# Slienteagle-wyb/tdmpc

Measured on AMD Instinct MI355X. Metric: plan-steps/sec (N=512, H=5, iters=6) at 1/2/4/8 MI355X vs CPU ref, higher is better.
Workload: dtype fp32

## Files before the change

### tdmpc_amd/csrc/tdmpc_kernels.hip

```cpp
#include <hip/hip_runtime.h>
#include <hiprand/hiprand_kernel.h>

#include <math.h>
#include <stdint.h>
#include <stdio.h>
#include <stdlib.h>
#include <string.h>
#include <unistd.h>

#include <algorithm>
#include <atomic>
#include <chrono>
#include <mutex>
#include <type_traits>
#include <vector>

#include "../../include/tdmpc_hip.h"

typedef float floatx16 __attribute__((ext_vector_type(16)));

#define DEVI __device__ __forceinline__

#ifdef TDMPC_STAMPS
__device__ unsigned long long* g_stamps;
// ... 180 lines not shown

constexpr int SPLIT_S = 4;
constexpr int SPLIT_MAX_ROWS = 4096;

struct Work {
    float* X;
    float* H1;
    float* H2;
    float2* st1;
    float2* st2;
    float* rpart;
    float* G;
    float* rlast;
    float* value;
    float* qv;
    float* z0c;
    float* pimu;
    float* zpart;
    float* rpart_s;
    int split_rows;
    float* z0;
    float* mean;
    float* stdv;
    float* enc_tmp;
    size_t x_stride;
    int xrows;
    char* p1;
    size_t p1_bytes;
    size_t total;
};

size_t pixel_act_floats(const Layout& w) {
    size_t m = 0;
    for (int i = 1; i <= 4; ++i) m = std::max(m, (size_t)w.nch * w.conv_hw[i] * w.conv_hw[i]);
    return m;
}

constexpr int P1_NG = 8;
constexpr int P1_WPG = 32;
constexpr int P1_RTM = 3;
constexpr int P1_ROWS = 32 * P1_RTM;
constexpr int P1_H1LD = 544;
constexpr unsigned P1_XCC_TAB = P1_NG * 256 + 256;
constexpr unsigned P1_SPIN_MAX = 400000;

struct P1Region {
// ... 51 lines not shown
    const size_t M = w.M;
    size_t o = 0;
    auto take = [&](size_t bytes) { size_t r = o; o += rup(bytes, 256); return base ? base + r : nullptr; };
    k->xrows = (int)rup(B * T, 32);
    k->x_stride = (size_t)k->xrows * w.Kx;
    k->X = (float*)take((H + 1) * k->x_stride * 4);
    k->H1 = (float*)take((size_t)k->xrows * 2 * M * 4);
    k->H2 = (float*)take((size_t)k->xrows * 2 * M * 4);
    k->st1 = (float2*)take(B * T * (2 * M / 64) * 8);
    k->st2 = (float2*)take(B * T * (2 * M / 64) * 8);
    k->rpart = (float*)take(B * T * (M / 32) * 4);
    k->G = (float*)take(B * T * 4);
    k->rlast = (float*)take(B * T * 4);
    k->value = (float*)take(B * T * 4);
    k->qv = (float*)take(2 * (size_t)k->xrows * 4);
    k->pimu = (float*)take((size_t)k->xrows * w.Ap * 4);
    k->z0c = (float*)take(B * 2 * M * 4);
    k->split_rows = std::min(k->xrows, SPLIT_MAX_ROWS);
    k->zpart = (float*)take((size_t)2 * SPLIT_S * k->split_rows * std::max(w.Lr, w.Ar) * 4);
    k->rpart_s = (float*)take((size_t)2 * SPLIT_S * k->split_rows * 4);
    k->z0 = (float*)take(B * w.Lp * 4);
    k->mean = (float*)take(B * H * w.A * 4);
    k->stdv = (float*)take(B * H * w.A * 4);
    k->enc_tmp = (float*)take(d->modality ? 2 * B * pixel_act_floats(w) * 4 : 256);
    k->p1_bytes = p1_dims_ok(d, w) && !extra ? p1_region(d, w).total : 0;
    k->p1 = k->p1_bytes ? (char*)take(k->p1_bytes) : nullptr;
    k->total = o;
}

size_t cem_lds_bytes(int T, int H, int K, int A) {
    const size_t nl = (T + 63) / 64;
    return nl * 64 * 8 + ((size_t)H * K * A + 64 + 4 * rup((size_t)H * A, 4) + 64 + 32) * 4;
}

bool check_dims(const tdmpc_dims* d) {
    if (!d) return false;
    if (d->num_samples <= 0 || d->num_pi < 0 || d->num_elites <= 0 || d->max_horizon <= 0 ||
        d->max_horizon > 16 || d->max_iterations <= 0 || d->max_batch <= 0) return false;
    const int T = d->num_samples + d->num_pi;
    if (d->num_elites > T || d->num_elites > 64 || T > 4096) return false;
    Layout w;
    if (!make_layout(d, &w)) return false;
    if (w.Kx > 1024 || w.M > 1024 || w.L > 1024 || w.A > 256 || w.E > 1024) return false;
    if (cem_lds_bytes(T, d->max_horizon, d->num_elites, w.A) > 160 * 1024) return false;
    return true;
}
// ... 1802 lines not shown
    const int e = row / a.eps_G, rr = row % a.eps_G;
    const float* ep = a.eps + (size_t)e * a.eps_env + a.eps_off + (size_t)rr * a.A;
    float o[4];
#pragma unroll
    for (int cc = 0; cc < 4; ++cc) {
        const int col = 4 * q + cc;
        float x = 0.f;
        if (col < a.A) {
            float sv = a.part[(size_t)row * a.n3 + col];
#pragma unroll
            for (int sl = 1; sl < SPLIT_S; ++sl) sv += a.part[((size_t)sl * a.prow + row) * a.n3 + col];
            const float muv = tanhf(sv + a.b3[col]);
            x = muv;
            if (a.min_std > 0.f) {
                const float ee = tclamp(fmul(ep[col], a.min_std), -0.3f, 0.3f);
                x = tclamp(fadd(muv, ee), a.lo, a.hi);
            }
        }
        o[cc] = x;
    }
    *(float4*)(a.Xo + (size_t)(xr >> 5) * a.x_ts + (size_t)q * 128 + (xr & 31) * 4) = make_float4(o[0], o[1], o[2], o[3]);
}

__global__ void __launch_bounds__(256) z0c_kernel(const float* W1, const float* b1, const float* z0, int Kx, int Ap,
                                                   int Lp, int k1c, int M, float* out) {
    const int e = blockIdx.x, p = blockIdx.y, n = blockIdx.z * 256 + threadIdx.x;
    if (n >= M) return;
    const int nn = p * M + n;
    const float* wrow = W1 + (size_t)(nn >> 5) * Kx * 32 + (nn & 31) * 4;
    float acc = 0.f;
#pragma unroll 8
    for (int kq = k1c >> 2; kq < Kx >> 2; ++kq) {
        const float4 w = *(const float4*)(wrow + kq * 128);
        const int zi = 4 * kq - Ap;
        const float* zr = z0 + (size_t)e * Lp;
        acc = fmaf(w.x, zi + 0 < Lp ? zr[zi + 0] : 0.f, acc);
        acc = fmaf(w.y, zi + 1 < Lp ? zr[zi + 1] : 0.f, acc);
        acc = fmaf(w.z, zi + 2 < Lp ? zr[zi + 2] : 0.f, acc);
        acc = fmaf(w.w, zi + 3 < Lp ? zr[zi + 3] : 0.f, acc);
    }
    out[((size_t)e * 2 + p) * M + n] = acc + b1[nn];
}

struct PiMuArgs {
    int rows; RowMap amap; RowMap mmap; const float* mu; int Ap, A; float* Xo; long x_ts;
    const float* eps; int eps_G; long eps_env; long eps_off; float min_std, lo, hi;
};

DEVI void pi_from_mu_item(const PiMuArgs& a, long i) {
    const int nq = a.Ap / 4;
    const int row = (int)(i / nq), q = (int)(i % nq);
    if (row >= a.rows) return;
    const int xr = map_row(a.amap, row);
    const int e = row / a.eps_G, rr = row % a.eps_G;
    const float* ep = a.eps + (size_t)e * a.eps_env + a.eps_off + (size_t)rr * a.A;
    const float4 m = *(const float4*)(a.mu + (size_t)map_row(a.mmap, row) * a.Ap + 4 * q);
    const float mv[4] = {m.x, m.y, m.z, m.w};
    float o[4];
#pragma unroll
    for (int cc = 0; cc < 4; ++cc) {
        const int col = 4 * q + cc;
        float x = 0.f;
        if (col < a.A) {
            x = mv[cc];
// ... 104 lines not shown
    __syncthreads();
    if (tid < 32 && row < a.rows) {
        float q[2];
        for (int p = 0; p < 2; ++p) {
            float s = 0.f;
            for (int i = 0; i < 16; ++i) s += red[p][i][r];
            q[p] = s + a.b3[p];
        }
        const float qm = (q[0] != q[0] || q[1] != q[1]) ? NAN : fminf(q[0], q[1]);
        const int x = map_row(a.map, row);
        a.value[x] = nan_to_num(fadd(a.G[x], fmul(a.disc, qm)));
    }
}


struct PrepArgs {
    float* X; size_t x_stride; int Kx, apq, lpq;
    int B, N, T, H, A;
    const float* mean; const float* stdv; int mstride;
    const float* eps; long eps_env; long eps_off;
    const float* z0;
    long n_zq, n_sq;
    PiMuArgs pm; long n_pm;
};

__global__ void __launch_bounds__(256) prep_kernel(const PrepArgs a) {
    const long total = a.n_zq + a.n_sq + a.n_pm;
    for (long it = (long)blockIdx.x * blockDim.x + threadIdx.x; it < total; it += (long)gridDim.x * blockDim.x) {
        if (it >= a.n_zq + a.n_sq) {
            pi_from_mu_item(a.pm, it - a.n_zq - a.n_sq);
        } else if (it < a.n_zq) {
            const int row = (int)(it % a.T);
            const long r2 = it / a.T;
            const int q = (int)(r2 % a.lpq), e = (int)(r2 / a.lpq);
            const int gr = e * a.T + row;
            *(float4*)(a.X + (size_t)(gr >> 5) * a.Kx * 32 + (size_t)(a.apq + q) * 128 + (gr & 31) * 4) =
                *(const float4*)(a.z0 + (size_t)e * a.lpq * 4 + q * 4);
        } else {
            long r2 = it - a.n_zq;
            const int n = (int)(r2 % a.N); r2 /= a.N;
            const int q = (int)(r2 % a.apq); r2 /= a.apq;
            const int t = (int)(r2 % a.H);
            const int e = (int)(r2 / a.H);
            const float* mt = a.mean + (size_t)e * a.mstride + (size_t)t * a.A;
            const float* sd = a.stdv + (size_t)e * a.mstride + (size_t)t * a.A;
            const float* ep = a.eps + (size_t)e * a.eps_env + a.eps_off + ((size_t)t * a.N + n) * a.A;
            float v[4];
#pragma unroll
            for (int k = 0; k < 4; ++k) {
                const int cc = q * 4 + k;
                v[k] = cc < a.A ? tclamp(fadd(mt[cc], fmul(sd[cc], ep[cc])), -1.f, 1.f) : 0.f;
            }
// ... 46 lines not shown
                        const float ep = a.eps[(size_t)e * a.eps_env + a.reuse_off + ((size_t)t * a.E + j) * a.A + cc];
                        x = tclamp(fadd(mt[cc], fmul(sd[cc], ep)), -1.f, 1.f);
                    }
                }
                v[k] = x;
            }
        }
        const int gr = e * a.Tw + row;
        *(float4*)(a.X + (size_t)t * a.x_stride + (size_t)(gr >> 5) * a.Kx * 32 + (size_t)q * 128 + (gr & 31) * 4) =
            make_float4(v[0], v[1], v[2], v[3]);
    }
}

struct CemArgs {
    int final_iter, iter, H, N, P, T, A, K, Kx, Hmax, I;
    int Tw, NE, pi_base;
    float* elite_store;
    const float* X; size_t x_stride;
    const float* value;
    const float* G; const float* qv; int q_ld; float discH;
    float* value_out;
    const float* rlast;
    float* mean; float* stdv;
    const float* eps; long eps_env; long eps_cem_off; long eps_iter; long eps_act_off;
    const double* u;
    float* prev_mean; int eval_mode;
    float temperature, momentum, omm, std_floor;
    const float* std_floor_p;
    float* action; float* metrics;
    float* elite_out; float* score_out; float* mean_out; float* std_out;
    int no_pick; float* reward_out;
    const int* pstatus; int* status;
};

DEVI uint32_t f2ord(float v) {
    const uint32_t u = __float_as_uint(v);
    return (u & 0x80000000u) ? ~u : (u | 0x80000000u);
}
DEVI float ord2f(uint32_t o) { return __uint_as_float((o & 0x80000000u) ? (o & 0x7fffffffu) : ~o); }
DEVI unsigned long long topk_key(float v, int i) {
    return ((unsigned long long)(~f2ord(v)) << 32) | (unsigned)i;
}
DEVI float key_value(unsigned long long k) { return ord2f(~(uint32_t)(k >> 32)); }

DEVI unsigned long long shfl_xor_u64(unsigned long long v, int m) {
    const unsigned lo = __shfl_xor((unsigned)v, m, 64), hi = __shfl_xor((unsigned)(v >> 32), m, 64);
// ... 2 lines not shown
DEVI unsigned long long wave_sort64(unsigned long long key, int lane) {
    for (int k = 2; k <= 64; k <<= 1)
        for (int j = k >> 1; j > 0; j >>= 1) {
            const unsigned long long o = shfl_xor_u64(key, j);
            const bool up = (lane & k) == 0, lower = (lane & j) == 0;
            key = (lower == up) ? (key < o ? key : o) : (key > o ? key : o);
        }
    return key;
}
DEVI unsigned long long wave_clean64(unsigned long long key, int lane) {
    for (int j = 32; j > 0; j >>= 1) {
        const unsigned long long o = shfl_xor_u64(key, j);
        key = ((lane & j) == 0) ? (key < o ? key : o) : (key > o ? key : o);
    }
    return key;
}
DEVI float wave_sum(float v) {
    for (int off = 32; off > 0; off >>= 1) v += __shfl_xor(v, off, 64);
    return v;
}

DEVI int cem_row(const CemArgs& a, int c) { return c < a.NE ? c : a.pi_base + (c - a.NE); }

__global__ void __launch_bounds__(1024) cem_kernel(const CemArgs a) {
    extern __shared__ __attribute__((aligned(16))) float sm[];
    const int e = blockIdx.x, tid = threadIdx.x, nt = blockDim.x, lane = tid & 63, wave = tid >> 6;
    const int nwv = nt >> 6;
    const int H = a.H, A = a.A, K = a.K, T = a.T, N = a.N;
    const int HA = H * A, HKA = H * K * A;
    const int NL = (T + 63) / 64;
    unsigned long long* key = (unsigned long long*)sm;
    float* EA = (float*)(key + (size_t)NL * 64);
    float* sc = EA + HKA;
    float* omean = sc + 64;
    float* smean = omean + 2 * rup(HA, 4);
    float* sstd = smean + rup(HA, 4);
    int* eidx = (int*)(sstd + rup(HA, 4));
    float* red = (float*)(eidx + 64);
    float* gmean = a.mean + (size_t)e * a.Hmax * A;
    float* gstd = a.stdv + (size_t)e * a.Hmax * A;
    const float* val = a.value + (size_t)e * a.Tw;

    for (int i = tid; i < HA; i += nt) omean[i] = gmean[i];
    for (int l = wave; l < NL; l += nwv) {
        const int i = l * 64 + lane;
        float v = 0.f;
        if (i < T) {
            const int row = cem_row(a, i);
            if (a.qv) {
                const size_t x = (size_t)e * a.Tw + row;
                v = qvalue(a.G[x], a.qv[x], a.qv[a.q_ld + x], a.discH);
                if (a.value_out) a.value_out[((size_t)e * a.I + a.iter) * a.Tw + i] = v;
            } else {
                v = val[row];
                if (a.value_out) a.value_out[((size_t)e * a.I + a.iter) * a.Tw + i] = v;
            }
        }
        const unsigned long long k = i < T ? topk_key(v, i) : ~0ull;
        key[(size_t)l * 64 + lane] = wave_sort64(k, lane);
    }
    __syncthreads();
    for (int stride = 1; stride < NL; stride <<= 1) {
        for (int l = wave * 2 * stride; l < NL; l += nwv * 2 * stride) {
            if (l + stride < NL) {
                const unsigned long long x = key[(size_t)l * 64 + lane];
                const unsigned long long y = key[(size_t)(l + stride) * 64 + 63 - lane];
                key[(size_t)l * 64 + lane] = wave_clean64(x < y ? x : y, lane);
            }
        }
        __syncthreads();
    }
    if (tid < K) eidx[tid] = (int)(key[tid] & 0xffffffffu);
    __syncthreads();
    for (int base = 0; base < HKA; base += 8 * nt) {
        float v[8];
#pragma unroll
        for (int u = 0; u < 8; ++u) {
            const int idx = base + tid + u * nt;
            if (idx < HKA) {
                const int t = idx / (K * A), k = (idx / A) % K, c = idx % A;
                v[u] = a.X[(size_t)t * a.x_stride + pidx((size_t)e * a.Tw + cem_row(a, eidx[k]), c, a.Kx)];
            }
        }
#pragma unroll
        for (int u = 0; u < 8; ++u) {
            const int idx = base + tid + u * nt;
            if (idx < HKA) EA[idx] = v[u];
        }
    }
    if (wave == 0) {
        const float v0 = key_value(key[0]);
        float s = 0.f;
        if (lane < K) s = expf(fmul(a.temperature, key_value(key[lane]) - v0));
        const float tot = wave_sum(s);
        s = lane < K ? __fdiv_rn(s, tot) : 0.f;
        if (lane < 64) sc[lane] = s;
        const float tot2 = wave_sum(s);
        if (lane == 0) red[0] = fadd(tot2, 1e-9f);
    }
    __syncthreads();
    const float den = red[0];
    const float std_floor = a.std_floor_p ? *a.std_floor_p : a.std_floor;
    for (int i = tid; i < HA; i += nt) {
        const int t = i / A, c = i % A;
        const float* ea = EA + (size_t)t * K * A + c;
        float s = 0.f;
        for (int k = 0; k < K; ++k) s = fadd(s, fmul(sc[k], ea[(size_t)k * A]));
        const float mu = __fdiv_rn(s, den);
        float v = 0.f;
        for (int k = 0; k < K; ++k) {
            const float dd = ea[(size_t)k * A] - mu;
            v = fadd(v, fmul(sc[k], fmul(dd, dd)));
        }
        const float sd = tclamp(sqrtf(__fdiv_rn(v, den)), std_floor, 2.f);
        const float nm = fadd(fmul(a.momentum, omean[i]), fmul(a.omm, mu));
        smean[i] = nm; sstd[i] = sd;
        gmean[i] = nm; gstd[i] = sd;
        if (a.mean_out) a.mean_out[((size_t)e * a.I + a.iter) * HA + i] = nm;
        if (a.std_out) a.std_out[((size_t)e * a.I + a.iter) * HA + i] = sd;
    }
    if (a.elite_store)
        for (int i = tid; i < HKA; i += nt) a.elite_store[(size_t)e * a.Hmax * a.K * A + i] = EA[i];
    if (!a.final_iter) return;
    const int pst = a.pstatus ? *a.pstatus : 0;
    if (pst && tid == 0 && a.status)
        __hip_atomic_fetch_or(a.status, pst, __ATOMIC_RELAXED, __HIP_MEMORY_SCOPE_AGENT);
    if (a.elite_out)
        for (int i = tid; i < HKA; i += nt) a.elite_out[(size_t)e * HKA + i] = EA[i];
    if (a.score_out && tid < K) a.score_out[(size_t)e * K + tid] = sc[tid];
    {
        float s = 0.f;
        for (int i = tid; i < T; i += nt) s += a.rlast[(size_t)e * a.Tw + cem_row(a, i)];
        s = wave_sum(s);
        if (lane == 0) red[1 + wave] = s;
    }
    __syncthreads();
    if (a.no_pick) {
        if (tid == 0) {
            float rs = 0.f;
            for (int w = 0; w < nwv; ++w) rs += red[1 + w];
            a.reward_out[e] = rs / (float)T;
        }
        return;
    }
    int* jsel = (int*)(red + 20);
    if (tid == 0) {
        double last = 0.0;
        for (int k = 0; k < K; ++k) last += (double)sc[k];
        const double u = a.u[e];
        double acc = 0.0;
        int j = K - 1;
        for (int k = 0; k < K; ++k) {
            acc += (double)sc[k];
            if (acc / last > u) { j = k; break; }
        }
        *jsel = j;
        float rs = 0.f;
        for (int w = 0; w < nwv; ++w) rs += red[1 + w];
        float cs = 0.f;
        for (int c = 0; c < A; ++c) cs += sstd[c];
        a.metrics[(size_t)e * 2 + 0] = pst ? __builtin_nanf("") : rs / (float)T;
        a.metrics[(size_t)e * 2 + 1] = pst ? __builtin_nanf("") : cs / (float)A;
    }
    __syncthreads();
    const int j = *jsel;
    for (int c = tid; c < A; c += nt) {
        float v = EA[(size_t)j * A + c];
        if (!a.eval_mode) v = fadd(v, fmul(sstd[c], a.eps[(size_t)e * a.eps_env + a.eps_act_off + c]));
        if (pst) v = __builtin_nanf("");
        a.action[(size_t)e * A + c] = v;
        if (a.elite_store) a.elite_store[(size_t)e * a.Hmax * a.K * A + (size_t)j * A + c] = v;
    }
    for (int i = tid; i < HA; i += nt) a.prev_mean[(size_t)e * H * A + i] = smean[i];
}

struct EncArgs {
    const float* x; long x_stride; int xdim;
    int E, L, Lp;
    const float* w1t; const float* b1;
    const float* w2t; const float* b2;
    float* z0;
    float* mean; float* stdv; const float* prev_mean; int warm, H, A, Hmax;
    const int* warm_flags;
    const float* ln_g; const float* ln_b;
    int warm_keep_last;
    float init_std;
};

DEVI void enc_matvec(const float* wt, const float* in, int nin, int nout, float* part, int tid, int nt) {
    const int np = nt / nout > 0 ? nt / nout : 1;
    const int j = tid % nout, p = tid / nout;
    float s = 0.f;
    if (p < np && j < nout) {
#pragma unroll 8
        for (int k = p; k < nin; k += np) s += wt[(size_t)k * nout + j] * in[k];
    }
// ... 211 lines not shown
#define LDS_FOR_EACH(X) X(2, 1, 2, 4, 32) X(3, 1, 2, 4, 32) X(1, 1, 2, 2, 32)
#define CHAIN_FOR_EACH(X)                                                                            \
    X(CH_STEP, 1, 8, 4, 8, 0) X(CH_STEP, 2, 8, 4, 8, 0) X(CH_STEP, 4, 8, 4, 8, 0)                     \
    X(CH_PI, 1, 8, 4, 8, 0) X(CH_PI, 2, 8, 4, 8, 0) X(CH_PI, 4, 8, 4, 8, 0)                           \
    X(CH_Q, 1, 8, 4, 8, 0) X(CH_Q, 2, 8, 4, 8, 0) X(CH_Q, 4, 8, 4, 8, 0)                              \
    X(CH_STEP, 2, 8, 2, X6_D3, 1) X(CH_STEP, 4, 4, 2, 2, 1) X(CH_PI, 2, 8, 2, X6_D3, 1)               \
    X(CH_PI, 4, 4, 2, 2, 1) X(CH_Q, 2, 8, 2, X6_D3, 1) X(CH_Q, 4, 4, 2, 2, 1)
#define CHAIN16_FOR_EACH(X)                                                                          \
    X(CH_STEP, 2, 4, 4, 0) X(CH_STEP, 4, 4, 4, 0) X(CH_PI, 2, 4, 4, 0) X(CH_PI, 4, 4, 4, 0)           \
    X(CH_Q, 2, 4, 4, 0) X(CH_Q, 4, 4, 4, 0)                                                           \
    X(CH_STEP, 4, 4, 4, 1) X(CH_PI, 4, 4, 4, 1) X(CH_Q, 4, 4, 4, 1)
#define SPLIT_FOR_EACH(X) X(4, 4, 1) X(4, 4, 0)
#define CONV_TILE_FOR_EACH(X) X(1) X(2) X(4)
#define PLAN1_FOR_EACH(X) X(4) X(6)

int init_attrs() {
    static int done = 0;
    if (done) return 0;
    int rc = 0;
#define LINEAR_ATTR(...) rc |= set_max_lds<linear_kernel<__VA_ARGS__>>();
    FOR_EACH_LINEAR(LINEAR_ATTR)
#undef LINEAR_ATTR
    rc |= set_max_lds<cem_kernel>();
#define PLAN1_ATTR(KS) rc |= set_max_lds<plan1_kernel<KS>>();
    PLAN1_FOR_EACH(PLAN1_ATTR)
#undef PLAN1_ATTR
#define WIDE_ATTR(...) rc |= set_max_lds<wide_step_kernel<__VA_ARGS__>>();
    WIDE_FOR_EACH(WIDE_ATTR)
#undef WIDE_ATTR
#define WIDE_HEADS_ATTR(...) rc |= set_max_lds<wide_heads_kernel<__VA_ARGS__>>();
    WIDE_HEADS_FOR_EACH(WIDE_HEADS_ATTR)
#undef WIDE_HEADS_ATTR
    rc |= set_max_lds<qstat_chol_kernel>();
#define CONV_ATTR(PX) rc |= set_max_lds<conv_tile_kernel<PX>>();
    CONV_TILE_FOR_EACH(CONV_ATTR)
#undef CONV_ATTR
#define LDS_ATTR(...) rc |= set_max_lds<linear_lds_kernel<__VA_ARGS__, true>>() | set_max_lds<linear_lds_kernel<__VA_ARGS__, false>>();
    LDS_FOR_EACH(LDS_ATTR)
#undef LDS_ATTR
#define CHAIN_ATTR(...) rc |= set_max_lds<chain_kernel<__VA_ARGS__>>();
    CHAIN_FOR_EACH(CHAIN_ATTR)
#undef CHAIN_ATTR
#define CHAIN16_ATTR(...) rc |= set_max_lds<chain16_kernel<__VA_ARGS__>>();
    CHAIN16_FOR_EACH(CHAIN16_ATTR)
#undef CHAIN16_ATTR
    if (rc) return TDMPC_E_HIP;
// ... 327 lines not shown
    f.n3 = w.Lr; f.L = w.L; f.Lp = w.Lp; f.b3d = c.pw + w.b3d; f.b3r = c.pw + w.b3r;
    f.Xo = Xt(c, t + 1); f.x_ts = (long)c.Kx * 32; f.out_q0 = w.Ap / 4;
    f.G = c.k.G; f.rlast = c.k.rlast; f.disc = disc; f.first = first; f.last = last;
    const long nth = (long)rows * (w.Lp / 4 + 1);
    hipLaunchKernelGGL(split_finish_kernel, dim3((unsigned)((nth + 255) / 256)), dim3(256), 0, c.s, f);
    HIPCHK(hipGetLastError());
    return 0;
}

int flush_split(const Ctx& c) {
    if (!c.split_pend) return 0;
    c.split_pend = 0;
    const int par = 1 - c.split_par;
    const size_t zs = (size_t)SPLIT_S * c.k.split_rows * std::max(c.w.Lr, c.w.Ar), rs = (size_t)SPLIT_S * c.k.split_rows;
    return split_finish(c, c.split_t, c.split_rows, c.split_map, c.k.zpart + par * zs, c.k.rpart_s + par * rs,
                        c.split_disc, c.split_first, 0);
}

int z0c_k1c(const Ctx& c) { return (int)rup(c.w.Ap, 16); }
bool z0c_eligible(const Ctx& c) {
    static const int v = [] { const char* e = getenv("TDMPC_Z0C"); return e ? atoi(e) : 1; }();
    return v && z0c_k1c(c) < (int)rup(c.Kx, 16);
}
int z0c_launch(const Ctx& c) {
    hipLaunchKernelGGL(z0c_kernel, dim3(c.B, 2, (c.M + 255) / 256), dim3(256), 0, c.s, c.pw + c.w.w1x, c.pw + c.w.b1x,
                       c.k.z0, c.Kx, c.w.Ap, c.w.Lp, z0c_k1c(c), c.M, c.k.z0c);
    HIPCHK(hipGetLastError());
    return 0;
}

unsigned long long* g_p1_stamps = nullptr;

int wide_g1(const Ctx& c, bool z0c) {
    return (int)rup(z0c ? z0c_k1c(c) : c.Kx, 32) / 32;
}
bool wide_instance(int g1, int nb3, int mode) {
#define WIDE_HAS(G1, NB3, MODE) if (g1 == G1 && nb3 == NB3 && mode == (MODE)) return true;
    WIDE_FOR_EACH(WIDE_HAS)
#undef WIDE_HAS
    return false;
}
bool use_wide(const Ctx& c, int rows, const RowMap& map, bool z0c) {
    static const int en = [] { const char* e = getenv("TDMPC_WIDE"); return e ? atoi(e) : 1; }();
    if (c.w.M != 512 || !use_x6(c) || !num_cus()) return false;
    if (c.path != TDMPC_PATH_AUTO && c.path != TDMPC_PATH_CHAIN && c.path != TDMPC_PATH_WIDE) return false;
    if (c.path != TDMPC_PATH_WIDE && !en) return false;
    if (rows % 16 || map.G % 16 || map.S % 16 || map.O % 16) return false;
    if (z0c && map.G % 128) return false;
    const int g1 = wide_g1(c, z0c), nb3 = (int)rup(c.w.L, 16) / 16, mode = g1 > 5 ? WS_XS : 0;
    if (!wide_instance(g1, nb3, mode) || (c.w.fold && !wide_instance(g1, nb3, mode | WS_OUTH))) return false;
    return c.path == TDMPC_PATH_WIDE || (rows + 127) / 128 * 2 >= num_cus();
// ... 274 lines not shown

PiMuArgs pimu_args(const Ctx& c, int rows, RowMap map, const float* eps, long eps_env, int eps_G, long eps_off,
                   float min_std, float* Xo = nullptr, const RowMap* mmap = nullptr) {
    PiMuArgs f;
    memset(&f, 0, sizeof f);
    f.rows = rows; f.amap = map; f.mmap = mmap ? *mmap : map; f.mu = c.k.pimu; f.Ap = c.w.Ap; f.A = c.w.A;
    f.Xo = Xo ? Xo : Xt(c, c.H); f.x_ts = (long)c.Kx * 32;
    f.eps = eps; f.eps_G = eps_G; f.eps_env = eps_env; f.eps_off = eps_off; f.min_std = min_std;
    f.lo = (float)(-1.0 + 1e-6); f.hi = (float)(1.0 - 1e-6);
    return f;
}

int policy_from_mu(const Ctx& c, int rows, RowMap map, const float* eps, long eps_env, int eps_G, long eps_off,
                   float min_std, float* Xo = nullptr, const RowMap* mmap = nullptr) {
    const PiMuArgs f = pimu_args(c, rows, map, eps, eps_env, eps_G, eps_off, min_std, Xo, mmap);
    const long nth = (long)rows * (c.w.Ap / 4);
    if (!nth) return 0;
    hipLaunchKernelGGL(pi_from_mu_kernel, dim3((unsigned)((nth + 255) / 256)), dim3(256), 0, c.s, f);
    HIPCHK(hipGetLastError());
    return 0;
}

int prep_launch(const Ctx& c, const float* noise, int sample_rows, long eps_env, long eps_off, const float* z0,
                const PiMuArgs* pm) {
    PrepArgs a;
    memset(&a, 0, sizeof a);
    a.X = c.k.X; a.x_stride = c.k.x_stride; a.Kx = c.Kx; a.apq = c.w.Ap / 4; a.lpq = c.w.Lp / 4;
    a.B = c.B; a.N = sample_rows; a.T = c.T; a.H = c.H; a.A = c.A;
    a.mean = c.k.mean; a.stdv = c.k.stdv; a.mstride = c.d->max_horizon * c.A;
    a.eps = noise; a.eps_env = eps_env; a.eps_off = eps_off;
    a.z0 = z0;
    a.n_zq = z0 ? (long)c.B * a.lpq * c.T : 0;
    a.n_sq = noise ? (long)c.B * c.H * a.apq * sample_rows : 0;
    if (pm) {
        a.pm = *pm;
        a.n_pm = (long)pm->rows * (pm->Ap / 4);
    }
    const long total = a.n_zq + a.n_sq + a.n_pm;
    if (!total) return 0;
    const int blocks = (int)std::min<long>((total + 255) / 256, 2048);
    hipLaunchKernelGGL(prep_kernel, dim3(blocks), dim3(256), 0, c.s, a);
    HIPCHK(hipGetLastError());
    return 0;
}
int prep(const Ctx& c, const float* noise, int iter, const float* z0, const PiMuArgs* pm = nullptr) {
    return prep_launch(c, noise, c.N, c.eps_env, c.eps_cem_off + (long)iter * c.eps_iter, z0, pm);
}

int q_chain(const Ctx& c, int rows, RowMap map, const float* X = nullptr, float* qo = nullptr, int q_ld = 0,
            bool fold = false) {
    const Layout& w = c.w;
    const int M = c.M;
    ChainArgs a = chain0(c, rows, map, c.H, c.Kx, 0, 2);
    if (X) a.X = X;
    if (fold && !a.x6) {
        snprintf(g_err, sizeof g_err, "folded Q: chain x6 kernels only");
        return TDMPC_E_DIMS;
    }
    for (int q = 0; q < 2; ++q) {
        ChainProb& p = a.p[q];
        p.W1 = c.pw + w.wq1x + (size_t)q * M * c.Kx; p.b1 = c.pw + w.bq1x + q * M;
        p.g1 = c.pw + w.g1 + q * M; p.be1 = c.pw + w.be1 + q * M;
        p.W2 = c.pw + w.wq2 + (size_t)q * M * M; p.b2 = c.pw + w.bq2 + q * M;
        p.g2 = c.pw + w.g2 + q * M; p.be2 = c.pw + w.be2 + q * M;
        p.w3v = c.pw + w.wq3 + q * M; p.b3v = c.pw + w.bq3 + q;
        if (a.x6) {
            p.X1 = x6p(c, X6_WQ1X) + q * x6_w1_rows_stride(c);
            p.X2 = x6p(c, X6_WQ2) + (size_t)q * (M / 32) * (M / 16) * 1536;
        }
// ... 333 lines not shown
    return init_attrs();
}

int resolve_path(int path, bool whole_plan) {
    if (path < 0 || path > TDMPC_PATH_WIDE) { snprintf(g_err, sizeof g_err, "bad path"); return -1; }
    if (path == TDMPC_PATH_CHAIN64) return TDMPC_PATH_CHAIN_X6;
    return path == TDMPC_PATH_PERSIST && !whole_plan ? TDMPC_PATH_AUTO : path;
}

int load_z0(const Ctx& c, const float* z0) {
    const int L = c.w.L;
    hipLaunchKernelGGL(zero_words_kernel, dim3(1), dim3(256), 0, c.s, (unsigned*)c.k.z0, (int)((size_t)c.B * c.w.Lp));
    HIPCHK(hipGetLastError());
    HIPCHK(hipMemcpy2DAsync(c.k.z0, c.w.Lp * 4, z0, L * 4, L * 4, c.B, hipMemcpyDeviceToDevice, c.s));
    return prep(c, nullptr, 0, c.k.z0);
}

template <class Prm>
CemArgs cem_args(const Ctx& c, const Prm* prm, const float* eps, const double* u, float* prev_mean, float* action,
                 float* metrics, float* value_out, float* mean_out, float* std_out) {
    CemArgs ca;
    memset(&ca, 0, sizeof ca);
    ca.H = c.H; ca.N = c.N; ca.P = c.P; ca.T = ca.Tw = ca.NE = c.T; ca.A = c.A; ca.K = c.d->num_elites; ca.Kx = c.Kx;
    ca.Hmax = c.d->max_horizon; ca.mean = c.k.mean; ca.stdv = c.k.stdv; ca.pstatus = pack_status(c);
    ca.X = c.k.X; ca.x_stride = c.k.x_stride; ca.value = c.k.value; ca.rlast = c.k.rlast;
    ca.eps = eps; ca.u = u; ca.prev_mean = prev_mean;
    ca.eval_mode = prm->eval_mode; ca.temperature = prm->temperature; ca.momentum = prm->momentum;
    ca.omm = prm->one_minus_momentum; ca.std_floor = prm->std_floor; ca.action = action; ca.metrics = metrics;
    ca.value_out = value_out; ca.mean_out = mean_out; ca.std_out = std_out; ca.status = prm->status;
    return ca;
}
void cem_args_qv(CemArgs& ca, const Ctx& c, float discH) {
    ca.G = c.k.G; ca.qv = c.k.qv; ca.q_ld = c.k.xrows; ca.discH = discH;
}

struct ToldStep {
    const Ctx& c;
    int operator()(int t, int rows, RowMap map, float disc, int first, int last, int defer) const {
        return step_next(c, t, rows, map, disc, first, last, defer);
    }
};

struct PlanFast {
    bool z0c;
    bool fold;
    bool wide_heads;
    bool pi_cache;
};

template <class Step>
int cem_run(Ctx& c, const Step& step, const PlanFast& f, const tdmpc_plan_params* prm, const float* noise,
            const double* u, float* prev_mean, float* action, float* metrics, float* elite_out, float* score_out,
            float* value_out, float* mean_out, float* std_out) {
    int rc;
    const int H = c.H, I = prm->iterations, B = c.B, N = c.N, P = c.P, T = c.T;
    if ((rc = prep(c, noise, 0, c.k.z0))) return rc;
    if (f.z0c) {
        if ((rc = z0c_launch(c))) return rc;
        c.z0c_ready = 1;
    }
    if (f.fold) {
        const RowMap rm0 = {N, T, 0};
        c.fold_ok = c.w.fold && H > 1 && use_wide(c, B * N, rm0, c.z0c_ready != 0) && use_wide(c, B * N, rm0, false);
        c.fold_heads = c.fold_ok && !f.wide_heads && use_x6(c) && use_chain(c, B * N, 1, CK_PI) &&
                       use_chain(c, B * N, 2, CK_Q) && (P == 0 || use_chain(c, B * P, 2, CK_Q));
        if (c.fold_heads && P > 0 && use_chain(c, B * P, 2, CK_STEP) && use_chain(c, B * P, 1, CK_PI)) {
            const ChainArgs probe = chain0(c, B * P, RowMap{P, T, N}, 0, c.Kx, 0, 2);
            c.fold_policy = probe.rb == 32 && probe.x6;
        }
    }

    const RowMap all = {T, T, 0}, pm = {P, T, N}, rm = {N, T, 0};
    if (P > 0) {
        for (int t = 0; t < H; ++t) {
            if ((rc = policy(c, t, B * P, pm, noise, c.eps_env, P, (long)t * P * c.A, prm->min_std, nullptr,
                             c.fold_policy && t >= 1)))
                return rc;
            if ((rc = step(t, B * T, all, prm->discount_pow[t], t == 0, t == H - 1, 0))) return rc;
        }
    }
    CemArgs ca = cem_args(c, prm, noise, u, prev_mean, action, metrics, value_out, mean_out, std_out);
    ca.I = I; ca.std_floor_p = prm->std_floor_dev; ca.elite_out = elite_out; ca.score_out = score_out;
    ca.eps_env = c.eps_env; ca.eps_cem_off = c.eps_cem_off; ca.eps_iter = c.eps_iter; ca.eps_act_off = c.eps_act_off;
    if (f.wide_heads || c.fold_heads || use_chain(c, B * T, 2, CK_Q)) cem_args_qv(ca, c, prm->discount_pow[H]);
    const size_t cem_lds = cem_lds_bytes(T, H, ca.K, c.A);

    const bool pi_cache = f.pi_cache && P > 0 && use_chain(c, B * T, 1, CK_PI);
    for (int i = 0; i < I; ++i) {
        const long toff = c.eps_cem_off + (long)i * c.eps_iter + c.eps_term_off;
        if (i > 0) {
            const PiMuArgs pmu = pimu_args(c, B * P, pm, noise, c.eps_env, P, toff + (long)N * c.A, prm->min_std);
            if ((rc = prep(c, noise, i, nullptr, f.wide_heads && P > 0 ? &pmu : nullptr))) return rc;
        }
        if (i > 0 || P == 0)
            for (int t = 0; t < H; ++t)
                if ((rc = step(t, B * N, rm, prm->discount_pow[t], t == 0, t == H - 1, 1))) return rc;
        if (f.wide_heads) {
            if (P > 0) {
                if (i == 0) rc = policy(c, H, B * P, pm, noise, c.eps_env, P, toff + (long)N * c.A, prm->min_std, c.k.pimu);
                if (rc || (rc = flush_split(c))) return rc;
            }
            if ((rc = terminal_wide(c, noise, toff, prm->min_std))) return rc;
        } else if (c.fold_heads) {
            if ((rc = policy(c, H, B * N, rm, noise, c.eps_env, N, toff, prm->min_std, nullptr, true))) return rc;
            if (P > 0) {
                if (i == 0 || !pi_cache)
                    rc = policy(c, H, B * P, pm, noise, c.eps_env, P, toff + (long)N * c.A, prm->min_std,
                                pi_cache ? c.k.pimu : nullptr, c.fold_policy != 0);
                else
                    rc = policy_from_mu(c, B * P, pm, noise, c.eps_env, P, toff + (long)N * c.A, prm->min_std);
                if (rc) return rc;
            }
            if ((rc = q_chain(c, B * N, rm, nullptr, nullptr, 0, true))) return rc;
            if (P > 0 && (rc = q_chain(c, B * P, pm, nullptr, nullptr, 0, c.fold_policy != 0))) return rc;
        } else if (pi_cache && i > 0) {
            if ((rc = policy(c, H, B * N, rm, noise, c.eps_env, N, toff, prm->min_std))) return rc;
            if ((rc = flush_split(c))) return rc;
            if ((rc = policy_from_mu(c, B * P, pm, noise, c.eps_env, P, toff + (long)N * c.A, prm->min_std)))
                return rc;
        } else if ((rc = policy(c, H, B * T, all, noise, c.eps_env, T, toff, prm->min_std,
                                pi_cache ? c.k.pimu : nullptr))) {
            return rc;
        }
        if (!f.wide_heads && !c.fold_heads && (rc = terminal_q(c, prm->discount_pow[H]))) return rc;
        ca.final_iter = i == I - 1;
        ca.iter = i;
        hipLaunchKernelGGL(cem_kernel, dim3(B), dim3(1024), cem_lds, c.s, ca);
        HIPCHK(hipGetLastError());
    }
    return 0;
}

bool icem_counts_ok(const tdmpc_icem_params* prm, const tdmpc_dims* d, const char* who) {
    const int H = prm->horizon, I = prm->iterations, N = d->num_samples, K = d->num_elites, P0 = prm->n_pi0;
    if (I <= 0 || I > 16) { snprintf(g_err, sizeof g_err, "%s: 1..16 iterations", who); return false; }
    if (P0 <= 0 || P0 > d->num_pi || prm->n_samples[0] != N) {
        snprintf(g_err, sizeof g_err, "%s: bad counts", who);
        return false;
    }
    for (int i = 0; i < I; ++i) {
        const int Ni = prm->n_samples[i], Pi = prm->n_pi[i], Ei = prm->n_elite[i];
        if (Ni <= 0 || Ni > N || Pi <= 0 || Pi > P0 || Ei < 0 || Ei > K || Ni + Ei + Pi < K ||
            (Ei > 0 && i == 0 && !prm->has_elites) ||
            (i == 0 && Ei > 0 && prm->elite_horizon != H && prm->elite_horizon != H - 1)) {
            snprintf(g_err, sizeof g_err, "%s: bad counts at iteration %d", who, i);
            return false;
        }
    }
    return true;
}
// ... 478 lines not shown
```

Measured before the change: 6184.

## Fuse CEM refit with next-iteration sample prep and fold z0c into prep kernel

Adds a cem_prep_kernel that runs the CEM refit redundantly across several blocks per environment and then writes the next iteration's sampled actions (and policy-from-mu rows) into X. This removes the separate prep launch between iterations. The mean/std buffers are double-buffered so the old stats can be reread, and elite actions are recomputed from the old mean/std and eps instead of read from X. The z0c kernel becomes an item range inside prep_kernel, and the top-k merge goes from a 2-way to a 4-way tree. The cost is duplicated refit work per slice and extra LDS for the old std.

```diff
diff --git a/tdmpc_amd/csrc/tdmpc_kernels.hip b/tdmpc_amd/csrc/tdmpc_kernels.hip
--- a/tdmpc_amd/csrc/tdmpc_kernels.hip
+++ b/tdmpc_amd/csrc/tdmpc_kernels.hip
@@ -226,6 +226,8 @@
     float* z0;
     float* mean;
     float* stdv;
+    float* mean2;
+    float* stdv2;
     float* enc_tmp;
     size_t x_stride;
     int xrows;
@@ -323,6 +325,8 @@
     k->z0 = (float*)take(B * w.Lp * 4);
     k->mean = (float*)take(B * H * w.A * 4);
     k->stdv = (float*)take(B * H * w.A * 4);
+    k->mean2 = (float*)take(B * H * w.A * 4);
+    k->stdv2 = (float*)take(B * H * w.A * 4);
     k->enc_tmp = (float*)take(d->modality ? 2 * B * pixel_act_floats(w) * 4 : 256);
     k->p1_bytes = p1_dims_ok(d, w) && !extra ? p1_region(d, w).total : 0;
     k->p1 = k->p1_bytes ? (char*)take(k->p1_bytes) : nullptr;
@@ -2171,24 +2175,24 @@
     *(float4*)(a.Xo + (size_t)(xr >> 5) * a.x_ts + (size_t)q * 128 + (xr & 31) * 4) = make_float4(o[0], o[1], o[2], o[3]);
 }
 
-__global__ void __launch_bounds__(256) z0c_kernel(const float* W1, const float* b1, const float* z0, int Kx, int Ap,
-                                                   int Lp, int k1c, int M, float* out) {
-    const int e = blockIdx.x, p = blockIdx.y, n = blockIdx.z * 256 + threadIdx.x;
-    if (n >= M) return;
-    const int nn = p * M + n;
-    const float* wrow = W1 + (size_t)(nn >> 5) * Kx * 32 + (nn & 31) * 4;
+struct Z0cArgs { const float* W1; const float* b1; const float* z0; int Kx, Ap, Lp, k1c, M; float* out; };
+
+DEVI void z0c_item(const Z0cArgs& a, long i) {
+    const int n = (int)(i % a.M), p = (int)(i / a.M % 2), e = (int)(i / (2 * a.M));
+    const int nn = p * a.M + n;
+    const float* wrow = a.W1 + (size_t)(nn >> 5) * a.Kx * 32 + (nn & 31) * 4;
+    const float* zr = a.z0 + (size_t)e * a.Lp;
     float acc = 0.f;
 #pragma unroll 8
-    for (int kq = k1c >> 2; kq < Kx >> 2; ++kq) {
+    for (int kq = a.k1c >> 2; kq < a.Kx >> 2; ++kq) {
         const float4 w = *(const float4*)(wrow + kq * 128);
-        const int zi = 4 * kq - Ap;
-        const float* zr = z0 + (size_t)e * Lp;
-        acc = fmaf(w.x, zi + 0 < Lp ? zr[zi + 0] : 0.f, acc);
-        acc = fmaf(w.y, zi + 1 < Lp ? zr[zi + 1] : 0.f, acc);
-        acc = fmaf(w.z, zi + 2 < Lp ? zr[zi + 2] : 0.f, acc);
-        acc = fmaf(w.w, zi + 3 < Lp ? zr[zi + 3] : 0.f, acc);
-    }
-    out[((size_t)e * 2 + p) * M + n] = acc + b1[nn];
+        const int zi = 4 * kq - a.Ap;
+        acc = fmaf(w.x, zi + 0 < a.Lp ? zr[zi + 0] : 0.f, acc);
+        acc = fmaf(w.y, zi + 1 < a.Lp ? zr[zi + 1] : 0.f, acc);
+        acc = fmaf(w.z, zi + 2 < a.Lp ? zr[zi + 2] : 0.f, acc);
+        acc = fmaf(w.w, zi + 3 < a.Lp ? zr[zi + 3] : 0.f, acc);
+    }
+    a.out[i] = acc + a.b1[nn];
 }
 
 struct PiMuArgs {
@@ -2339,12 +2343,16 @@
     const float* z0;
     long n_zq, n_sq;
     PiMuArgs pm; long n_pm;
+    Z0cArgs zc; long n_zc;
 };
 
 __global__ void __launch_bounds__(256) prep_kernel(const PrepArgs a) {
-    const long total = a.n_zq + a.n_sq + a.n_pm;
-    for (long it = (long)blockIdx.x * blockDim.x + threadIdx.x; it < total; it += (long)gridDim.x * blockDim.x) {
-        if (it >= a.n_zq + a.n_sq) {
+    const long total = a.n_zc + a.n_zq + a.n_sq + a.n_pm;
+    for (long i = (long)blockIdx.x * blockDim.x + threadIdx.x; i < total; i += (long)gridDim.x * blockDim.x) {
+        const long it = i - a.n_zc;
+        if (it < 0) {
+            z0c_item(a.zc, i);
+        } else if (it >= a.n_zq + a.n_sq) {
             pi_from_mu_item(a.pm, it - a.n_zq - a.n_sq);
         } else if (it < a.n_zq) {
             const int row = (int)(it % a.T);
@@ -2437,6 +2445,9 @@
     float* value_out;
     const float* rlast;
     float* mean; float* stdv;
+    const float* mean_old; const float* std_old;
+    int fused, apq;
+    float* Xw; PiMuArgs pm; int pm_env;
     const float* eps; long eps_env; long eps_cem_off; long eps_iter; long eps_act_off;
     const double* u;
     float* prev_mean; int eval_mode;
@@ -2485,26 +2496,61 @@
 
 DEVI int cem_row(const CemArgs& a, int c) { return c < a.NE ? c : a.pi_base + (c - a.NE); }
 
-__global__ void __launch_bounds__(1024) cem_kernel(const CemArgs a) {
-    extern __shared__ __attribute__((aligned(16))) float sm[];
-    const int e = blockIdx.x, tid = threadIdx.x, nt = blockDim.x, lane = tid & 63, wave = tid >> 6;
+struct CemLds {
+    unsigned long long* key;
+    float* EA;
+    float* sc;
+    float* omean; float* ostd;
+    float* smean; float* sstd;
+    int* eidx;
+    float* red;
+};
+DEVI CemLds cem_lds(float* sm, const CemArgs& a) {
+    const int HA = a.H * a.A;
+    CemLds L;
+    L.key = (unsigned long long*)sm;
+    L.EA = (float*)(L.key + (size_t)((a.T + 63) / 64) * 64);
+    L.sc = L.EA + a.H * a.K * a.A;
+    L.omean = L.sc + 64;
+    L.ostd = L.omean + rup(HA, 4);
+    L.smean = L.ostd + rup(HA, 4);
+    L.sstd = L.smean + rup(HA, 4);
+    L.eidx = (int*)(L.sstd + rup(HA, 4));
+    L.red = (float*)(L.eidx + 64);
+    return L;
+}
+
+struct CemEarly { float std_floor, rsum; int pst; double u; };
+DEVI CemEarly cem_early(const CemArgs& a, int e, bool writer) {
+    CemEarly y;
+    y.std_floor = a.std_floor_p ? *a.std_floor_p : a.std_floor;
+    y.rsum = 0.f; y.pst = 0; y.u = 0.0;
+    if (a.final_iter && writer) {
+        y.pst = a.pstatus ? *a.pstatus : 0;
+        for (int i = threadIdx.x; i < a.T; i += blockDim.x) y.rsum += a.rlast[(size_t)e * a.Tw + cem_row(a, i)];
+        if (threadIdx.x == 0 && !a.no_pick) y.u = a.u[e];
+    }
+    return y;
+}
+
+DEVI void cem_refit(const CemArgs& a, const CemLds& L, const CemEarly& y, int e, bool writer) {
+    const int tid = threadIdx.x, nt = blockDim.x, lane = tid & 63, wave = tid >> 6;
     const int nwv = nt >> 6;
     const int H = a.H, A = a.A, K = a.K, T = a.T, N = a.N;
     const int HA = H * A, HKA = H * K * A;
     const int NL = (T + 63) / 64;
-    unsigned long long* key = (unsigned long long*)sm;
-    float* EA = (float*)(key + (size_t)NL * 64);
-    float* sc = EA + HKA;
-    float* omean = sc + 64;
-    float* smean = omean + 2 * rup(HA, 4);
-    float* sstd = smean + rup(HA, 4);
-    int* eidx = (int*)(sstd + rup(HA, 4));
-    float* red = (float*)(eidx + 64);
+    unsigned long long* key = L.key;
+    float *EA = L.EA, *sc = L.sc, *omean = L.omean, *smean = L.smean, *sstd = L.sstd, *red = L.red;
+    int* eidx = L.eidx;
     float* gmean = a.mean + (size_t)e * a.Hmax * A;
     float* gstd = a.stdv + (size_t)e * a.Hmax * A;
     const float* val = a.value + (size_t)e * a.Tw;
-
-    for (int i = tid; i < HA; i += nt) omean[i] = gmean[i];
+    float* value_out = writer ? a.value_out : nullptr;
+
+    for (int i = tid; i < HA; i += nt) {
+        omean[i] = a.mean_old[(size_t)e * a.Hmax * A + i];
+        if (a.fused) L.ostd[i] = a.std_old[(size_t)e * a.Hmax * A + i];
+    }
     for (int l = wave; l < NL; l += nwv) {
         const int i = l * 64 + lane;
         float v = 0.f;
@@ -2513,28 +2559,29 @@
             if (a.qv) {
                 const size_t x = (size_t)e * a.Tw + row;
                 v = qvalue(a.G[x], a.qv[x], a.qv[a.q_ld + x], a.discH);
-                if (a.value_out) a.value_out[((size_t)e * a.I + a.iter) * a.Tw + i] = v;
             } else {
                 v = val[row];
-                if (a.value_out) a.value_out[((size_t)e * a.I + a.iter) * a.Tw + i] = v;
             }
+            if (value_out) value_out[((size_t)e * a.I + a.iter) * a.Tw + i] = v;
         }
         const unsigned long long k = i < T ? topk_key(v, i) : ~0ull;
         key[(size_t)l * 64 + lane] = wave_sort64(k, lane);
     }
     __syncthreads();
-    for (int stride = 1; stride < NL; stride <<= 1) {
-        for (int l = wave * 2 * stride; l < NL; l += nwv * 2 * stride) {
-            if (l + stride < NL) {
-                const unsigned long long x = key[(size_t)l * 64 + lane];
-                const unsigned long long y = key[(size_t)(l + stride) * 64 + 63 - lane];
-                key[(size_t)l * 64 + lane] = wave_clean64(x < y ? x : y, lane);
+    for (int stride = 1; stride < NL; stride <<= 2) {
+        for (int l = wave * 4 * stride; l < NL; l += nwv * 4 * stride) {
+            unsigned long long x = key[(size_t)l * 64 + lane];
+            for (int j = 1; j < 4 && l + j * stride < NL; ++j) {
+                const unsigned long long o = key[(size_t)(l + j * stride) * 64 + 63 - lane];
+                x = wave_clean64(x < o ? x : o, lane);
             }
+            key[(size_t)l * 64 + lane] = x;
         }
         __syncthreads();
     }
     if (tid < K) eidx[tid] = (int)(key[tid] & 0xffffffffu);
     __syncthreads();
+    const float* eps_it = a.fused ? a.eps + (size_t)e * a.eps_env + a.eps_cem_off + (size_t)a.iter * a.eps_iter : nullptr;
     for (int base = 0; base < HKA; base += 8 * nt) {
         float v[8];
 #pragma unroll
@@ -2542,7 +2589,12 @@
             const int idx = base + tid + u * nt;
             if (idx < HKA) {
                 const int t = idx / (K * A), k = (idx / A) % K, c = idx % A;
-                v[u] = a.X[(size_t)t * a.x_stride + pidx((size_t)e * a.Tw + cem_row(a, eidx[k]), c, a.Kx)];
+                const int cand = eidx[k];
+                if (a.fused && cand < N)
+                    v[u] = tclamp(fadd(omean[t * A + c], fmul(L.ostd[t * A + c], eps_it[((size_t)t * N + cand) * A + c])),
+                                  -1.f, 1.f);
+                else
+                    v[u] = a.X[(size_t)t * a.x_stride + pidx((size_t)e * a.Tw + cem_row(a, cand), c, a.Kx)];
             }
         }
 #pragma unroll
@@ -2563,7 +2615,7 @@
     }
     __syncthreads();
     const float den = red[0];
-    const float std_floor = a.std_floor_p ? *a.std_floor_p : a.std_floor;
+    const float std_floor = y.std_floor;
     for (int i = tid; i < HA; i += nt) {
         const int t = i / A, c = i % A;
         const float* ea = EA + (size_t)t * K * A + c;
@@ -2578,23 +2630,29 @@
         const float sd = tclamp(sqrtf(__fdiv_rn(v, den)), std_floor, 2.f);
         const float nm = fadd(fmul(a.momentum, omean[i]), fmul(a.omm, mu));
         smean[i] = nm; sstd[i] = sd;
+        if (!writer) continue;
         gmean[i] = nm; gstd[i] = sd;
         if (a.mean_out) a.mean_out[((size_t)e * a.I + a.iter) * HA + i] = nm;
         if (a.std_out) a.std_out[((size_t)e * a.I + a.iter) * HA + i] = sd;
     }
-    if (a.elite_store)
+    if (a.elite_store && writer)
         for (int i = tid; i < HKA; i += nt) a.elite_store[(size_t)e * a.Hmax * a.K * A + i] = EA[i];
-    if (!a.final_iter) return;
-    const int pst = a.pstatus ? *a.pstatus : 0;
+}
+
+DEVI void cem_pick(const CemArgs& a, const CemLds& L, const CemEarly& y, int e) {
+    const int tid = threadIdx.x, nt = blockDim.x, lane = tid & 63, wave = tid >> 6;
+    const int nwv = nt >> 6;
+    const int H = a.H, A = a.A, K = a.K, T = a.T;
+    const int HA = H * A, HKA = H * K * A;
+    float *EA = L.EA, *sc = L.sc, *smean = L.smean, *sstd = L.sstd, *red = L.red;
+    const int pst = y.pst;
     if (pst && tid == 0 && a.status)
         __hip_atomic_fetch_or(a.status, pst, __ATOMIC_RELAXED, __HIP_MEMORY_SCOPE_AGENT);
     if (a.elite_out)
         for (int i = tid; i < HKA; i += nt) a.elite_out[(size_t)e * HKA + i] = EA[i];
     if (a.score_out && tid < K) a.score_out[(size_t)e * K + tid] = sc[tid];
     {
-        float s = 0.f;
-        for (int i = tid; i < T; i += nt) s += a.rlast[(size_t)e * a.Tw + cem_row(a, i)];
-        s = wave_sum(s);
+        const float s = wave_sum(y.rsum);
         if (lane == 0) red[1 + wave] = s;
     }
     __syncthreads();
@@ -2610,7 +2668,7 @@
     if (tid == 0) {
         double last = 0.0;
         for (int k = 0; k < K; ++k) last += (double)sc[k];
-        const double u = a.u[e];
+        const double u = y.u;
         double acc = 0.0;
         int j = K - 1;
         for (int k = 0; k < K; ++k) {
@@ -2635,6 +2693,69 @@
         if (a.elite_store) a.elite_store[(size_t)e * a.Hmax * a.K * A + (size_t)j * A + c] = v;
     }
     for (int i = tid; i < HA; i += nt) a.prev_mean[(size_t)e * H * A + i] = smean[i];
+}
+
+__global__ void __launch_bounds__(1024) cem_kernel(const CemArgs a) {
+    extern __shared__ __attribute__((aligned(16))) float sm[];
+    const int e = blockIdx.x;
+    const CemLds L = cem_lds(sm, a);
+    const CemEarly y = cem_early(a, e, true);
+    cem_refit(a, L, y, e, true);
+    if (a.final_iter) cem_pick(a, L, y, e);
+}
+
+constexpr int FILL_U = 2;
+
+DEVI void fill_load(const CemArgs& a, const float* ep, int j, float (&v)[4]) {
+    const int n = j % a.N, q = (j / a.N) % a.apq, t = j / (a.N * a.apq);
+#pragma unroll
+    for (int k = 0; k < 4; ++k) {
+        const int cc = q * 4 + k;
+        v[k] = cc < a.A ? ep[((size_t)t * a.N + n) * a.A + cc] : 0.f;
+    }
+}
+DEVI void fill_store(const CemArgs& a, const CemLds& L, int e, int j, const float (&ev)[4]) {
+    const int n = j % a.N, q = (j / a.N) % a.apq, t = j / (a.N * a.apq);
+    float v[4];
+#pragma unroll
+    for (int k = 0; k < 4; ++k) {
+        const int cc = q * 4 + k;
+        v[k] = cc < a.A ? tclamp(fadd(L.smean[t * a.A + cc], fmul(L.sstd[t * a.A + cc], ev[k])), -1.f, 1.f) : 0.f;
+    }
+    const int gr = e * a.Tw + n;
+    *(float4*)(a.Xw + (size_t)t * a.x_stride + (size_t)(gr >> 5) * a.Kx * 32 + (size_t)q * 128 + (gr & 31) * 4) =
+        make_float4(v[0], v[1], v[2], v[3]);
+}
+
+__global__ void __launch_bounds__(1024) cem_prep_kernel(const CemArgs a) {
+    extern __shared__ __attribute__((aligned(16))) float sm[];
+    const int e = blockIdx.x, slice = blockIdx.y, tid = threadIdx.x;
+    const int stride = gridDim.y * blockDim.x, j0 = slice * blockDim.x + tid;
+    const bool writer = slice == 0;
+    const CemLds L = cem_lds(sm, a);
+    const CemEarly y = cem_early(a, e, writer);
+    const int n_sq = a.final_iter ? 0 : a.H * a.apq * a.N;
+    const float* ep = a.eps + (size_t)e * a.eps_env + a.eps_cem_off + (size_t)(a.iter + 1) * a.eps_iter;
+    float ev[FILL_U][4];
+#pragma unroll
+    for (int u = 0; u < FILL_U; ++u)
+        if (j0 + u * stride < n_sq) fill_load(a, ep, j0 + u * stride, ev[u]);
+    cem_refit(a, L, y, e, writer);
+    if (a.final_iter) {
+        if (writer) cem_pick(a, L, y, e);
+        return;
+    }
+    __syncthreads();
+    for (int base = j0; base < n_sq; base += FILL_U * stride) {
+#pragma unroll
+        for (int u = 0; u < FILL_U; ++u) {
+            const int j = base + u * stride;
+            if (j >= n_sq) break;
+            if (base != j0) fill_load(a, ep, j, ev[u]);
+            fill_store(a, L, e, j, ev[u]);
+        }
+    }
+    for (int j = j0; j < a.pm_env; j += stride) pi_from_mu_item(a.pm, (long)e * a.pm_env + j);
 }
 
 struct EncArgs {
@@ -2892,6 +3013,7 @@
     FOR_EACH_LINEAR(LINEAR_ATTR)
 #undef LINEAR_ATTR
     rc |= set_max_lds<cem_kernel>();
+    rc |= set_max_lds<cem_prep_kernel>();
 #define PLAN1_ATTR(KS) rc |= set_max_lds<plan1_kernel<KS>>();
     PLAN1_FOR_EACH(PLAN1_ATTR)
 #undef PLAN1_ATTR
@@ -3265,11 +3387,8 @@
     static const int v = [] { const char* e = getenv("TDMPC_Z0C"); return e ? atoi(e) : 1; }();
     return v && z0c_k1c(c) < (int)rup(c.Kx, 16);
 }
-int z0c_launch(const Ctx& c) {
-    hipLaunchKernelGGL(z0c_kernel, dim3(c.B, 2, (c.M + 255) / 256), dim3(256), 0, c.s, c.pw + c.w.w1x, c.pw + c.w.b1x,
-                       c.k.z0, c.Kx, c.w.Ap, c.w.Lp, z0c_k1c(c), c.M, c.k.z0c);
-    HIPCHK(hipGetLastError());
-    return 0;
+Z0cArgs z0c_args(const Ctx& c) {
+    return Z0cArgs{c.pw + c.w.w1x, c.pw + c.w.b1x, c.k.z0, c.Kx, c.w.Ap, c.w.Lp, z0c_k1c(c), c.M, c.k.z0c};
 }
 
 unsigned long long* g_p1_stamps = nullptr;
@@ -3590,7 +3709,7 @@
 }
 
 int prep_launch(const Ctx& c, const float* noise, int sample_rows, long eps_env, long eps_off, const float* z0,
-                const PiMuArgs* pm) {
+                const PiMuArgs* pm, const Z0cArgs* zc = nullptr) {
     PrepArgs a;
     memset(&a, 0, sizeof a);
     a.X = c.k.X; a.x_stride = c.k.x_stride; a.Kx = c.Kx; a.apq = c.w.Ap / 4; a.lpq = c.w.Lp / 4;
@@ -3604,15 +3723,20 @@
         a.pm = *pm;
         a.n_pm = (long)pm->rows * (pm->Ap / 4);
     }
-    const long total = a.n_zq + a.n_sq + a.n_pm;
+    if (zc) {
+        a.zc = *zc;
+        a.n_zc = (long)c.B * 2 * zc->M;
+    }
+    const long total = a.n_zc + a.n_zq + a.n_sq + a.n_pm;
     if (!total) return 0;
     const int blocks = (int)std::min<long>((total + 255) / 256, 2048);
     hipLaunchKernelGGL(prep_kernel, dim3(blocks), dim3(256), 0, c.s, a);
     HIPCHK(hipGetLastError());
     return 0;
 }
-int prep(const Ctx& c, const float* noise, int iter, const float* z0, const PiMuArgs* pm = nullptr) {
-    return prep_launch(c, noise, c.N, c.eps_env, c.eps_cem_off + (long)iter * c.eps_iter, z0, pm);
+int prep(const Ctx& c, const float* noise, int iter, const float* z0, const PiMuArgs* pm = nullptr,
+         const Z0cArgs* zc = nullptr) {
+    return prep_launch(c, noise, c.N, c.eps_env, c.eps_cem_off + (long)iter * c.eps_iter, z0, pm, zc);
 }
 
 int q_chain(const Ctx& c, int rows, RowMap map, const float* X = nullptr, float* qo = nullptr, int q_ld = 0,
@@ -3992,7 +4116,8 @@
     CemArgs ca;
     memset(&ca, 0, sizeof ca);
     ca.H = c.H; ca.N = c.N; ca.P = c.P; ca.T = ca.Tw = ca.NE = c.T; ca.A = c.A; ca.K = c.d->num_elites; ca.Kx = c.Kx;
-    ca.Hmax = c.d->max_horizon; ca.mean = c.k.mean; ca.stdv = c.k.stdv; ca.pstatus = pack_status(c);
+    ca.Hmax = c.d->max_horizon; ca.mean_old = ca.mean = c.k.mean; ca.std_old = ca.stdv = c.k.stdv;
+    ca.pstatus = pack_status(c);
     ca.X = c.k.X; ca.x_stride = c.k.x_stride; ca.value = c.k.value; ca.rlast = c.k.rlast;
     ca.eps = eps; ca.u = u; ca.prev_mean = prev_mean;
     ca.eval_mode = prm->eval_mode; ca.temperature = prm->temperature; ca.momentum = prm->momentum;
@@ -4018,17 +4143,24 @@
     bool pi_cache;
 };
 
+bool cem_fuse_on() {
+    const char* e = getenv("TDMPC_CEM_FUSE");
+    return !e || atoi(e) != 0;
+}
+int cem_slices(const Ctx& c) {
+    const long items = (long)c.H * (c.w.Ap / 4) * c.N;
+    return (int)std::max<long>(1, std::min<long>(std::max(num_cus(), 1) / c.B, (items + 255) / 256));
+}
+
 template <class Step>
 int cem_run(Ctx& c, const Step& step, const PlanFast& f, const tdmpc_plan_params* prm, const float* noise,
             const double* u, float* prev_mean, float* action, float* metrics, float* elite_out, float* score_out,
             float* value_out, float* mean_out, float* std_out) {
     int rc;
     const int H = c.H, I = prm->iterations, B = c.B, N = c.N, P = c.P, T = c.T;
-    if ((rc = prep(c, noise, 0, c.k.z0))) return rc;
-    if (f.z0c) {
-        if ((rc = z0c_launch(c))) return rc;
-        c.z0c_ready = 1;
-    }
+    const Z0cArgs zc = z0c_args(c);
+    if ((rc = prep(c, noise, 0, c.k.z0, nullptr, f.z0c ? &zc : nullptr))) return rc;
+    if (f.z0c) c.z0c_ready = 1;
     if (f.fold) {
         const RowMap rm0 = {N, T, 0};
         c.fold_ok = c.w.fold && H > 1 && use_wide(c, B * N, rm0, c.z0c_ready != 0) && use_wide(c, B * N, rm0, false);
@@ -4054,13 +4186,19 @@
     ca.eps_env = c.eps_env; ca.eps_cem_off = c.eps_cem_off; ca.eps_iter = c.eps_iter; ca.eps_act_off = c.eps_act_off;
     if (f.wide_heads || c.fold_heads || use_chain(c, B * T, 2, CK_Q)) cem_args_qv(ca, c, prm->discount_pow[H]);
     const size_t cem_lds = cem_lds_bytes(T, H, ca.K, c.A);
+    const bool fuse = cem_fuse_on();
+    ca.fused = fuse; ca.Xw = c.k.X; ca.apq = c.w.Ap / 4;
 
     const bool pi_cache = f.pi_cache && P > 0 && use_chain(c, B * T, 1, CK_PI);
     for (int i = 0; i < I; ++i) {
         const long toff = c.eps_cem_off + (long)i * c.eps_iter + c.eps_term_off;
-        if (i > 0) {
-            const PiMuArgs pmu = pimu_args(c, B * P, pm, noise, c.eps_env, P, toff + (long)N * c.A, prm->min_std);
-            if ((rc = prep(c, noise, i, nullptr, f.wide_heads && P > 0 ? &pmu : nullptr))) return rc;
+        auto pmu = [&](int j) {
+            return pimu_args(c, B * P, pm, noise, c.eps_env, P, toff + (j - i) * c.eps_iter + (long)N * c.A, prm->min_std);
+        };
+        const bool ride = f.wide_heads && P > 0;
+        if (i > 0 && !fuse) {
+            const PiMuArgs pi = pmu(i);
+            if ((rc = prep(c, noise, i, nullptr, ride ? &pi : nullptr))) return rc;
         }
         if (i > 0 || P == 0)
             for (int t = 0; t < H; ++t)
@@ -4095,7 +4233,15 @@
         if (!f.wide_heads && !c.fold_heads && (rc = terminal_q(c, prm->discount_pow[H]))) return rc;
         ca.final_iter = i == I - 1;
         ca.iter = i;
-        hipLaunchKernelGGL(cem_kernel, dim3(B), dim3(1024), cem_lds, c.s, ca);
+        if (fuse) {
+            ca.mean_old = i & 1 ? c.k.mean2 : c.k.mean; ca.std_old = i & 1 ? c.k.stdv2 : c.k.stdv;
+            ca.mean = i & 1 ? c.k.mean : c.k.mean2; ca.stdv = i & 1 ? c.k.stdv : c.k.stdv2;
+            ca.pm_env = 0;
+            if (ride && !ca.final_iter) { ca.pm = pmu(i + 1); ca.pm_env = P * (c.w.Ap / 4); }
+            hipLaunchKernelGGL(cem_prep_kernel, dim3(B, ca.final_iter ? 1 : cem_slices(c)), dim3(1024), cem_lds, c.s, ca);
+        } else {
+            hipLaunchKernelGGL(cem_kernel, dim3(B), dim3(1024), cem_lds, c.s, ca);
+        }
         HIPCHK(hipGetLastError());
     }
     return 0;
```

Result: no change. 6230 (median of 6 runs) (+0.7%).
